# intel-aero/aero-optical-flow

Measured on AMD Instinct MI355X. Metric: frame-pairs/s (640x480, 8x8 SAD, +-4 search), higher is better.
Workload: dtype u8

## Files before the change

aero-optical-flow_amd/csrc/aof_batch.cpp:

```cpp
#include <cerrno>

#include "aof_batch_plan.hpp"
#include "aof_ctx.hpp"

using namespace aof;

namespace {

struct Timed {
    aof_ctx *ctx; int id; hipStream_t s; bool on; int slot;
    Timed(aof_ctx *c, int k, hipStream_t st)
        : ctx(c), id(k), s(st), on(c->prof.on && !c->capturing && ((c->prof.mask >> k) & 1u)),
          slot((int)(c->prof.count[k] % AOF_PROFILE_RING))
    {
        if (on) (void)hipEventRecord(ctx->prof.ev[id][slot][0], s);
    }
    ~Timed() { if (on) { (void)hipEventRecord(ctx->prof.ev[id][slot][1], s); ctx->prof.count[id]++; } }
};

VoteMem vote_mem(const aof_ctx *ctx) { return {ctx->votes.mem, kVoteStride, ctx->h_fault, ctx->votes.deadline_ticks}; }

int launch_lane8(aof_ctx *ctx, SearchArgs a, const FlowTail &tail, hipStream_t s, bool *reduced)
{
    hipStreamCaptureStatus status = hipStreamCaptureStatusNone;
    const Capture cap = hipStreamIsCapturing(s, &status) != hipSuccess ? CAPTURE_UNKNOWN
                        : status == hipStreamCaptureStatusNone         ? CAPTURE_NONE
                                                                       : CAPTURE_ACTIVE;
    const VoteMem vm = vote_mem(ctx);
    Lane8Launch l = choose_lane8(ctx->cfg, ctx->adapt, a, cap, vm, ctx->votes.pairs, ctx->votes.separate, ctx->votes.captured);
    a.prune = l.prune;
    const bool eager = cap == CAPTURE_NONE;
    if (l.fused && eager && ctx->votes.used && ctx->votes.stream != s && hipStreamWaitEvent(s, ctx->votes.done, 0) != hipSuccess)
// ... 167 lines not shown
```

aero-optical-flow_amd/csrc/aof_flow_small.hpp:

```cpp
#pragma once

#include "aof_device.hpp"
#include "aof_internal.hpp"
#include "aof_reduce.hpp"
#include "aof_refine.hpp"
#include "aof_sad.hpp"
#include "aof_small_plan.hpp"

namespace aof {

namespace {

__device__ __forceinline__ uint4 lds_bytes16(const uint8_t *frame, int off)
{
    const uint32_t *q = reinterpret_cast<const uint32_t *>(frame) + (off >> 2);
    const uint32_t sh = (uint32_t)off & 3u;
    const uint32_t q0 = q[0], q1 = q[1], q2 = q[2], q3 = q[3], q4 = q[4];
    return make_uint4(__builtin_amdgcn_alignbyte(q1, q0, sh), __builtin_amdgcn_alignbyte(q2, q1, sh),
                      __builtin_amdgcn_alignbyte(q3, q2, sh), __builtin_amdgcn_alignbyte(q4, q3, sh));
}
__device__ __forceinline__ void lds_bytes8(const uint8_t *frame, int off, uint32_t (&out)[2])
{
    const uint32_t *q = reinterpret_cast<const uint32_t *>(frame) + (off >> 2);
    const uint32_t sh = (uint32_t)off & 3u;
// ... 309 lines not shown
}

inline size_t small_lds_bytes(const SmallArgs &a) { return small_plan_make(a).lds; }

template <typename... Params, typename... Args>
inline int launch_small_class(void (*fn)(Params...), uint32_t grid, const SmallArgs &sm, void *stream, const Args &...args)
{
    const SmallPlan plan = small_plan_make(sm);
    if (plan.verdict != SMALL_OK) return (int)hipErrorInvalidValue;
    const size_t lds = plan.lds;
    if (plan.attr) {
        const hipError_t e = hipFuncSetAttribute(reinterpret_cast<const void *>(fn),
                                                 hipFuncAttributeMaxDynamicSharedMemorySize, (int)(kSmallLdsLimit - kSmallStaticLds));
        if (e != hipSuccess) return (int)e;
    }
    hipLaunchKernelGGL(fn, dim3(grid), dim3(kThreads), lds, static_cast<hipStream_t>(stream), args...);
    return (int)hipGetLastError();
}

}

}
```

aero-optical-flow_amd/csrc/k_coarse.hip:

```cpp
#include <cstdint>

#include "aof_coarse_plan.hpp"
#include "aof_device.hpp"
#include "aof_internal.hpp"
#include "aof_lab_hooks.hpp"
#include "aof_reduce.hpp"
#include "aof_sad.hpp"

namespace aof {

namespace {

constexpr int kThreads = 512;
constexpr int kUnroll = 4;
constexpr uint32_t kGated = 0xFFFFFFFEu;
constexpr uint32_t kOpen = 0xFFFFFFFFu;
constexpr int kMaxBins = 64;
constexpr int kNonTemporal = 2;
constexpr int kScratch = 8;
static_assert(kThreads == kCoarseThreads && kUnroll == kCoarseUnroll && kMaxBins == kCoarseMaxBins && kScratch == kCoarseScratch,
              "the kernel and its plan agree on the workgroup, the batches and the histograms");

__device__ __forceinline__ void lds_barrier()
{
// ... 257 lines not shown
        k.stagger_ticks = plan.stagger_ticks;
    }
    const size_t lds = plan.lds;
    const int64_t wgs = plan.wgs;
#ifdef AOF_LAB_COARSE_WS
    {
        int rc = 0;
        if (lab_launch_coarse_ws(k, wgs, lds, stream, &rc)) return rc;
    }
#endif
    {
        const hipError_t e = hipFuncSetAttribute(reinterpret_cast<const void *>(k_coarse),
                                                 hipFuncAttributeMaxDynamicSharedMemorySize, (int)kCoarseLdsLimit);
        if (e != hipSuccess) return (int)e;
    }
    hipLaunchKernelGGL(k_coarse, dim3((uint32_t)wgs), dim3(kThreads), lds, static_cast<hipStream_t>(stream), k);
    return (int)hipGetLastError();
}

}
```

aero-optical-flow_amd/csrc/k_cols8_flow_f.hip:

```cpp
#include "aof_cols8_kernels.hpp"
#include "aof_lane8_launch.hpp"

namespace aof {

int launch_k_flow_lane8_cols_f(const SearchArgs &a, const ColsPlan &plan, const PruneReport &rep, const ColsVotes &cv, uint32_t grid, int threads,
                               void *stream)
{
    hipLaunchKernelGGL((k_flow_lane8_cols<false>), dim3(grid), dim3(threads), 0, static_cast<hipStream_t>(stream), a, plan, rep, cv);
    return (int)hipGetLastError();
}

}
```

aero-optical-flow_amd/csrc/k_cols8_flow_t.hip:

```cpp
#include "aof_cols8_kernels.hpp"
#include "aof_lane8_launch.hpp"

namespace aof {

int launch_k_flow_lane8_cols_t(const SearchArgs &a, const ColsPlan &plan, const PruneReport &rep, const ColsVotes &cv, uint32_t grid, int threads,
                               void *stream)
{
    hipLaunchKernelGGL((k_flow_lane8_cols<true>), dim3(grid), dim3(threads), 0, static_cast<hipStream_t>(stream), a, plan, rep, cv);
    return (int)hipGetLastError();
}

}
```

aero-optical-flow_amd/csrc/k_cols8_search_f.hip:

```cpp
#include "aof_cols8_kernels.hpp"
#include "aof_lane8_launch.hpp"

namespace aof {

int launch_k_search_lane8_cols_f(const SearchArgs &a, const ColsPlan &plan, const PruneReport &rep, uint32_t wgs, int threads, void *stream)
{
    hipLaunchKernelGGL((k_search_lane8_cols<false>), dim3(wgs), dim3(threads), 0, static_cast<hipStream_t>(stream), a, plan, rep);
    return (int)hipGetLastError();
}

}
```

aero-optical-flow_amd/csrc/k_cols8_search_t.hip:

```cpp
#include "aof_cols8_kernels.hpp"
#include "aof_lane8_launch.hpp"

namespace aof {

int launch_k_search_lane8_cols_t(const SearchArgs &a, const ColsPlan &plan, const PruneReport &rep, uint32_t wgs, int threads, void *stream)
{
    hipLaunchKernelGGL((k_search_lane8_cols<true>), dim3(wgs), dim3(threads), 0, static_cast<hipStream_t>(stream), a, plan, rep);
    return (int)hipGetLastError();
}

}
```

aero-optical-flow_amd/csrc/k_lane8_flat_ff.hip:

```cpp
#include "aof_lane8_kernels.hpp"
#include "aof_lane8_launch.hpp"

namespace aof {

int launch_k_flow_lane8_flat_ff(const SearchArgs &a, uint32_t items, uint32_t search_wgs, uint32_t grid, int threads, const FlowTail &t,
                                const VoteMem &v, void *stream)
{
    hipLaunchKernelGGL((k_flow_lane8_flat<false, false>), dim3(grid), dim3(threads), 0, static_cast<hipStream_t>(stream), a, items, search_wgs, t, v);
    return (int)hipGetLastError();
}

}
```

aero-optical-flow_amd/csrc/k_lane8_flat_ft.hip:

```cpp
#include "aof_lane8_kernels.hpp"
#include "aof_lane8_launch.hpp"

namespace aof {

int launch_k_flow_lane8_flat_ft(const SearchArgs &a, uint32_t items, uint32_t search_wgs, uint32_t grid, int threads, const FlowTail &t,
                                const VoteMem &v, void *stream)
{
    hipLaunchKernelGGL((k_flow_lane8_flat<false, true>), dim3(grid), dim3(threads), 0, static_cast<hipStream_t>(stream), a, items, search_wgs, t, v);
    return (int)hipGetLastError();
}

}
```

aero-optical-flow_amd/csrc/k_lane8_flat_tf.hip:

```cpp
#include "aof_lane8_kernels.hpp"
#include "aof_lane8_launch.hpp"

namespace aof {

int launch_k_flow_lane8_flat_tf(const SearchArgs &a, uint32_t items, uint32_t search_wgs, uint32_t grid, int threads, const FlowTail &t,
                                const VoteMem &v, void *stream)
{
    hipLaunchKernelGGL((k_flow_lane8_flat<true, false>), dim3(grid), dim3(threads), 0, static_cast<hipStream_t>(stream), a, items, search_wgs, t, v);
    return (int)hipGetLastError();
}

}
```

aero-optical-flow_amd/csrc/k_lane8_flat_tt.hip:

```cpp
#include "aof_lane8_kernels.hpp"
#include "aof_lane8_launch.hpp"

namespace aof {

int launch_k_flow_lane8_flat_tt(const SearchArgs &a, uint32_t items, uint32_t search_wgs, uint32_t grid, int threads, const FlowTail &t,
                                const VoteMem &v, void *stream)
{
    hipLaunchKernelGGL((k_flow_lane8_flat<true, true>), dim3(grid), dim3(threads), 0, static_cast<hipStream_t>(stream), a, items, search_wgs, t, v);
    return (int)hipGetLastError();
}

}
```

aero-optical-flow_amd/csrc/k_lane8_group_f.hip:

```cpp
#include "aof_lane8_kernels.hpp"
#include "aof_lane8_launch.hpp"

namespace aof {

int launch_k_flow_lane8_f(const SearchArgs &a, const FlowTail &t, int ppw, uint32_t wgs, size_t lds, void *stream)
{
    hipLaunchKernelGGL((k_flow_lane8<false>), dim3(wgs), dim3(kThreads), lds, static_cast<hipStream_t>(stream), a, t, ppw);
    return (int)hipGetLastError();
}

}
```

aero-optical-flow_amd/csrc/k_lane8_group_t.hip:

```cpp
#include "aof_lane8_kernels.hpp"
#include "aof_lane8_launch.hpp"

namespace aof {

int launch_k_flow_lane8_t(const SearchArgs &a, const FlowTail &t, int ppw, uint32_t wgs, size_t lds, void *stream)
{
    hipLaunchKernelGGL((k_flow_lane8<true>), dim3(wgs), dim3(kThreads), lds, static_cast<hipStream_t>(stream), a, t, ppw);
    return (int)hipGetLastError();
}

}
```

aero-optical-flow_amd/csrc/k_lane8_pruned_f.hip:

```cpp
#include "aof_lane8_kernels.hpp"
#include "aof_lane8_launch.hpp"

namespace aof {

int launch_k_search_lane8_pruned_f(const SearchArgs &a, uint32_t items, uint32_t wgs, int spw, const PruneReport &rep, void *stream)
{
    hipLaunchKernelGGL((k_search_lane8_pruned<false>), dim3(wgs), dim3(kThreads), 0, static_cast<hipStream_t>(stream), a, items, wgs, spw, rep);
    return (int)hipGetLastError();
}

}
```

aero-optical-flow_amd/csrc/k_lane8_pruned_t.hip:

```cpp
#include "aof_lane8_kernels.hpp"
#include "aof_lane8_launch.hpp"

namespace aof {

int launch_k_search_lane8_pruned_t(const SearchArgs &a, uint32_t items, uint32_t wgs, int spw, const PruneReport &rep, void *stream)
{
    hipLaunchKernelGGL((k_search_lane8_pruned<true>), dim3(wgs), dim3(kThreads), 0, static_cast<hipStream_t>(stream), a, items, wgs, spw, rep);
    return (int)hipGetLastError();
}

}
```

aero-optical-flow_amd/csrc/k_lane8_search_ff.hip:

```cpp
#include "aof_lane8_kernels.hpp"
#include "aof_lane8_launch.hpp"

namespace aof {

int launch_k_search_lane8_ff(const SearchArgs &a, uint32_t items, uint32_t wgs, int threads, void *stream)
{
    hipLaunchKernelGGL((k_search_lane8<false, false>), dim3(wgs), dim3(threads), 0, static_cast<hipStream_t>(stream), a, items, wgs, 1);
    return (int)hipGetLastError();
}

}
```

aero-optical-flow_amd/csrc/k_lane8_search_ft.hip:

```cpp
#include "aof_lane8_kernels.hpp"
#include "aof_lane8_launch.hpp"

namespace aof {

int launch_k_search_lane8_ft(const SearchArgs &a, uint32_t items, uint32_t wgs, int threads, void *stream)
{
    hipLaunchKernelGGL((k_search_lane8<false, true>), dim3(wgs), dim3(threads), 0, static_cast<hipStream_t>(stream), a, items, wgs, 1);
    return (int)hipGetLastError();
}

}
```

aero-optical-flow_amd/csrc/k_lane8_search_tf.hip:

```cpp
#include "aof_lane8_kernels.hpp"
#include "aof_lane8_launch.hpp"

namespace aof {

int launch_k_search_lane8_tf(const SearchArgs &a, uint32_t items, uint32_t wgs, int threads, void *stream)
{
    hipLaunchKernelGGL((k_search_lane8<true, false>), dim3(wgs), dim3(threads), 0, static_cast<hipStream_t>(stream), a, items, wgs, 1);
    return (int)hipGetLastError();
}

}
```

aero-optical-flow_amd/csrc/k_lane8_search_tt.hip:

```cpp
#include "aof_lane8_kernels.hpp"
#include "aof_lane8_launch.hpp"

namespace aof {

int launch_k_search_lane8_tt(const SearchArgs &a, uint32_t items, uint32_t wgs, int threads, void *stream)
{
    hipLaunchKernelGGL((k_search_lane8<true, true>), dim3(wgs), dim3(threads), 0, static_cast<hipStream_t>(stream), a, items, wgs, 1);
    return (int)hipGetLastError();
}

}
```

aero-optical-flow_amd/csrc/k_pyramid.hip:

```cpp
#include "aof_coarse_plan.hpp"
#include "aof_device.hpp"
#include "aof_internal.hpp"

namespace aof {

namespace {

constexpr int kThreads = 256;
static_assert(kThreads == kPyramidThreads, "the kernels and their plan agree on the workgroup");

__device__ __forceinline__ void publish_sums(const PyramidArgs &a, int64_t unit, int frame, uint32_t sum0, uint32_t sum1)
{
    if (!a.sequence) {
        atomicAdd(&a.sums[unit * 4 + frame * 2 + 0], sum0);
        atomicAdd(&a.sums[unit * 4 + frame * 2 + 1], sum1);
        return;
    }
    if (unit < a.n_pairs - 1) {
        atomicAdd(&a.sums[unit * 4 + 0], sum0);
        atomicAdd(&a.sums[unit * 4 + 1], sum1);
    }
    if (unit > 0) {
        atomicAdd(&a.sums[(unit - 1) * 4 + 2], sum0);
        atomicAdd(&a.sums[(unit - 1) * 4 + 3], sum1);
// ... 82 lines not shown
}

__global__ __launch_bounds__(kThreads) void k_zero_words(uint32_t *words, int64_t count)
{
    const int64_t i = (int64_t)blockIdx.x * kThreads + threadIdx.x;
    if (i < count) words[i] = 0;
}

}

int launch_zero_words(uint32_t *words, int64_t count, void *stream)
{
    if (count <= 0) return 0;
    const int64_t wgs = (count + kThreads - 1) / kThreads;
    if (wgs > 0x7FFFFFFF) return (int)hipErrorInvalidValue;
    hipLaunchKernelGGL(k_zero_words, dim3((uint32_t)wgs), dim3(kThreads), 0, static_cast<hipStream_t>(stream), words, count);
    return (int)hipGetLastError();
}

int launch_pyramid(const PyramidArgs &a, void *stream)
{
    if (a.n_pairs == 0) return 0;
    hipStream_t s = static_cast<hipStream_t>(stream);
    const PyramidPlan plan = pyramid_plan_make(a.w, a.h, a.pair_stride, reinterpret_cast<uintptr_t>(a.prev), reinterpret_cast<uintptr_t>(a.cur),
                                               a.sequence, a.n_pairs, a.sums != nullptr);
    if (a.sums) {
        const int rc = launch_zero_words(a.sums, plan.zero_words, stream);
        if (rc) return rc;
    }
    if (plan.total > 0x7FFFFFFF) return (int)hipErrorInvalidValue;
    if (plan.vec)
        hipLaunchKernelGGL(k_pyramid_vec, dim3((uint32_t)plan.total), dim3(kThreads), 0, s, a, plan.rows_per_strip, plan.nstrips);
    else
        hipLaunchKernelGGL(k_pyramid_scalar, dim3((uint32_t)plan.total), dim3(kThreads), 0, s, a, plan.nstrips);
    return (int)hipGetLastError();
}

}
```

aero-optical-flow_amd/csrc/k_reduce.hip:

```cpp
#include "aof_device.hpp"
#include "aof_internal.hpp"
#include "aof_reduce.hpp"

namespace aof {

namespace {

constexpr int kThreads = 256;
constexpr int kMaxHist = 256;
constexpr int64_t kMidPairs = 1024;
constexpr int64_t kWidePairs = 512;

template <int GROUP, int kThreads = 256>
__global__ __launch_bounds__(kThreads) void k_reduce(ReduceArgs a)
{
    constexpr int kGroups = kThreads / GROUP;
    __shared__ uint32_t s_hist[kGroups][2][kMaxHist];
    __shared__ int s_sums[kGroups][3];
    const int grp = (int)threadIdx.x / GROUP, tid = (int)threadIdx.x % GROUP;
    const int64_t pair = (int64_t)blockIdx.x * kGroups + grp;
    if (GROUP < kThreads && pair >= a.n_pairs) return;
    auto sync = [] { if (GROUP == kThreads) __syncthreads(); else __builtin_amdgcn_wave_barrier(); };
    uint32_t (*hist)[kMaxHist] = s_hist[grp];
    int *sums = s_sums[grp];
    const int centre = 2 * a.tail.range + 1, n = 2 * centre + 1;
    for (int k = tid; k < n; k += GROUP) { hist[0][k] = 0; hist[1][k] = 0; }
    if (tid < 3) sums[tid] = 0;
    sync();

    if (a.parts) {
        const uint32_t *parts = a.parts + (size_t)pair * a.nstrips * (size_t)(2 * n);
        for (int k = tid; k < 2 * n; k += GROUP) {
            uint32_t v = 0;
            for (int st = 0; st < a.nstrips; st++) v += parts[(size_t)st * (2 * n) + k];
            const int axis = k >= n, bin = k - axis * n;
            hist[axis][bin] = v;
// ... 125 lines not shown
        wave_vote(hist[1], 2 * r.dy + hy + centre, ok);
    }
    __syncthreads();
    uint32_t *out = a.chunk_parts + ((size_t)pair * chunks + chunk) * (size_t)(2 * n);
    for (int k = tid; k < 2 * n; k += kThreads) out[k] = k < n ? hist[0][k] : hist[1][k - n];
}

}

int launch_reduce(const ReduceArgs &a, void *stream)
{
    if (a.n_pairs == 0) return 0;
    if (a.n_pairs > 0x7FFFFFFF) return (int)hipErrorInvalidValue;
    const int chunks = a.parts ? 0 : reduce_chunks(a.tail.nblocks);
    if (chunks > 0 && a.chunk_parts && a.n_pairs * chunks <= 0x7FFFFFFF) {
        hipLaunchKernelGGL(k_reduce_chunk, dim3((uint32_t)(a.n_pairs * chunks)), dim3(kThreads), 0,
                           static_cast<hipStream_t>(stream), a, chunks);
        ReduceArgs b = a;
        b.parts = a.chunk_parts;
        b.nstrips = chunks;
        hipLaunchKernelGGL(k_reduce<kThreads>, dim3((uint32_t)a.n_pairs), dim3(kThreads), 0,
                           static_cast<hipStream_t>(stream), b);
        return (int)hipGetLastError();
    }
    if (a.tail.nblocks <= 256 && !a.parts)
        hipLaunchKernelGGL(k_reduce<64>, dim3((uint32_t)((a.n_pairs + 3) / 4)), dim3(kThreads), 0,
                           static_cast<hipStream_t>(stream), a);
    else if (a.n_pairs <= kWidePairs && a.tail.nblocks >= 2048 && !a.parts)
        hipLaunchKernelGGL((k_reduce<1024, 1024>), dim3((uint32_t)a.n_pairs), dim3(1024), 0,
                           static_cast<hipStream_t>(stream), a);
    else if (a.n_pairs <= kMidPairs && a.tail.nblocks >= 2048 && !a.parts)
        hipLaunchKernelGGL((k_reduce<512, 512>), dim3((uint32_t)a.n_pairs), dim3(512), 0,
                           static_cast<hipStream_t>(stream), a);
    else
        hipLaunchKernelGGL(k_reduce<kThreads>, dim3((uint32_t)a.n_pairs), dim3(kThreads), 0,
                           static_cast<hipStream_t>(stream), a);
    return (int)hipGetLastError();
}

}
```

aero-optical-flow_amd/csrc/k_refine.hip:

```cpp
#include "aof_device.hpp"
#include "aof_internal.hpp"
#include "aof_refine.hpp"

namespace aof {

namespace {

constexpr int kRefineThreads = 256;

template <int NW>
__global__ __launch_bounds__(kRefineThreads) void k_refine(SearchArgs a, int64_t items)
{
    constexpr int B = 4 * NW;
    const int64_t item = (int64_t)blockIdx.x * kRefineThreads + threadIdx.x;
    if (item >= items) return;
    const int nb = a.grid.blocks();
    const int64_t pair = item / nb;
    const int blk = (int)(item - pair * nb);
    const aof_block rec = __builtin_bit_cast(
        aof_block, reinterpret_cast<const uint32_t *>(a.blocks)[pair * nb + blk]);
    uint8_t *out = a.subdirs + pair * nb + blk;
    if (rec.sad == AOF_SAD_SKIPPED || (uint32_t)rec.sad >= (uint32_t)a.value_threshold) {
        *out = 8;
        return;
// ... 41 lines not shown
    });
    const int subdir = st.direction(rec.sad);
    *out = (uint8_t)subdir;
}

}

int launch_refine(const SearchArgs &a, void *stream)
{
    if (a.n_pairs == 0 || !a.subdirs) return 0;
    const int64_t items = a.n_pairs * a.grid.blocks();
    const int64_t wgs = (items + kRefineThreads - 1) / kRefineThreads;
    if (wgs > 0x7FFFFFFF) return (int)hipErrorInvalidValue;
    const dim3 grid((uint32_t)wgs);
    if (a.tile == 8)
        hipLaunchKernelGGL(k_refine<2>, grid, dim3(kRefineThreads), 0, static_cast<hipStream_t>(stream), a, items);
    else if (a.tile == 16)
        hipLaunchKernelGGL(k_refine<4>, grid, dim3(kRefineThreads), 0, static_cast<hipStream_t>(stream), a, items);
    else
        return (int)hipErrorInvalidValue;
    return (int)hipGetLastError();
}

}
```

aero-optical-flow_amd/csrc/k_search_generic.hip:

```cpp
#include "aof_device.hpp"
#include "aof_internal.hpp"

namespace aof {

namespace {

constexpr int kMaxTile = 16, kMaxSearch = 8;
constexpr int kMaxWin = kMaxTile + 2 * kMaxSearch + 2;
constexpr int kMaxPitch = (kMaxWin + 3) / 4 * 4;

__global__ __launch_bounds__(64) void k_search_generic(SearchArgs a)
{
    __shared__ __attribute__((aligned(16))) uint8_t s_ref[kMaxTile * kMaxTile];
    __shared__ __attribute__((aligned(16))) uint8_t s_win[kMaxPitch * kMaxWin + 16];

    const int lane = threadIdx.x;
    const int blk = blockIdx.x;
    const int64_t pair = blockIdx.y + (int64_t)blockIdx.z * gridDim.y;
    if (pair >= a.n_pairs) return;
    const int B = a.tile, S = a.search, m = a.subpixel ? 1 : 0;
    const int bx = blk % a.grid.nx, by = blk / a.grid.nx;
    const int i = a.grid.x0 + bx * a.grid.step_x, j = a.grid.y0 + by * a.grid.step_y;
    int px = 0, py = 0;
    if (a.pred) { px = a.pred[pair].pred_x; py = a.pred[pair].pred_y; }
// ... 100 lines not shown
        }
    }
    if (lane == 0) {
        *out = rec;
        if (out_sd) *out_sd = (uint8_t)subdir;
    }
}

}

int launch_search_generic(const SearchArgs &a, void *stream)
{
    if (a.n_pairs == 0) return 0;
    const int64_t gy = a.n_pairs < 32768 ? a.n_pairs : 32768;
    const int64_t gz = (a.n_pairs + gy - 1) / gy;
    hipLaunchKernelGGL(k_search_generic, dim3((uint32_t)a.grid.blocks(), (uint32_t)gy, (uint32_t)gz),
                       dim3(64), 0, static_cast<hipStream_t>(stream), a);
    return (int)hipGetLastError();
}

}
```

aero-optical-flow_amd/csrc/k_search_tile16.hip:

```cpp
#include "aof_device.hpp"
#include "aof_internal.hpp"
#include "aof_refine.hpp"
#include "aof_sad.hpp"
#include "aof_tile16_plan.hpp"

namespace aof {

namespace {

constexpr int kBoundRows = 2;
constexpr uint32_t kFullOverBound = 6;
constexpr uint32_t kMaxSurvivorsPct = 35;
constexpr uint32_t kFullOverOneRow = 12;
constexpr uint32_t kMaxOneRowSurvivorsPct = 4;
constexpr uint32_t kMaxFourRowSurvivorsPct = 40, kMaxEightRowSurvivorsPct = 10;
constexpr uint32_t kMaxSeparationForDeeperLook = 450;
constexpr int kRefineParts = 4;

template <int NR, int STEP>
__device__ __forceinline__ void sum_item(const uint8_t *s_prev, const uint8_t *s_cur, int W, int dyi, int bx, int xs,
                                         int first, u64 (&acc)[4], uint32_t &acc16, int delta = 0)
{
    uint32_t ref[NR][4];
#pragma unroll
// ... 496 lines not shown
constexpr uint32_t kForcedVerdictPattern = 0x5A5A00u;
__global__ __launch_bounds__(kFillThreads) void k_tile16_fill_verdicts(uint32_t *hints, int64_t n_pairs, Tile16Verdicts f)
{
    const int64_t i = (int64_t)blockIdx.x * kFillThreads + threadIdx.x;
    if (i < n_pairs) hints[i] = (uint32_t)f.v[i % f.count] | kForcedVerdictPattern;
}

}

int launch_search_tile16(const SearchArgs &a, void *stream, const Tile16Verdicts &forced)
{
    if (a.n_pairs == 0) return 0;
    const Tile16Plan p = tile16_plan(a, forced.count);
    if (p.refused) return (int)hipErrorInvalidValue;
    if (p.front == TILE16_FRONT_FILL) {
        hipLaunchKernelGGL(k_tile16_fill_verdicts, dim3((uint32_t)p.front_wgs), dim3(kFillThreads), 0, static_cast<hipStream_t>(stream), a.hints,
                           a.n_pairs, forced);
    } else if (p.front == TILE16_FRONT_PROBE) {
        hipLaunchKernelGGL(k_tile16_probe, dim3((uint32_t)p.front_wgs), dim3(kProbeThreads), 0, static_cast<hipStream_t>(stream), a, a.hints,
                           p.stx, p.sty);
    }
    if (p.front != TILE16_FRONT_NONE) {
        const hipError_t e = hipGetLastError();
        if (e != hipSuccess) return (int)e;
    }
    SearchArgs k = a;
    k.div_nx = fastdiv_make((uint32_t)a.grid.nx);
    void (*fn)(SearchArgs, uint32_t) =
        p.refine ? (p.prune ? k_search_tile16<true, true> : k_search_tile16<false, true>)
                 : (p.prune ? k_search_tile16<true, false> : k_search_tile16<false, false>);
    if (p.attr) {
        hipError_t e = hipFuncSetAttribute(reinterpret_cast<const void *>(fn), hipFuncAttributeMaxDynamicSharedMemorySize, (int)p.lds);
        if (e != hipSuccess) return (int)e;
    }
    hipLaunchKernelGGL(fn, dim3((uint32_t)p.total), dim3(kTile16Threads), p.lds, static_cast<hipStream_t>(stream), k, (uint32_t)p.total);
    return (int)hipGetLastError();
}

}
```

Measured before the change: 7.266 million.

## Route launches through profiling-aware wrapper and add bin-based per-pair reduce path

Adds a launch_kernel wrapper that, when profiling is active, records start/stop events inside the kernel launch via hipExtLaunchKernelGGL instead of issuing separate hipEventRecord calls, and converts all launch sites to it. Separately adds a reduce_pair_bins path in k_reduce for the full-workgroup case, voting into per-lane x/y bins with a weighted fast path when all four records in a quad agree. This is meant to avoid the shared-memory histogram work when the search range is small. The change also disables profiling during stream capture.

After: 7.427 million (median of 6 runs). 2.2% higher.

```diff
diff --git a/aero-optical-flow_amd/csrc/aof_batch.cpp b/aero-optical-flow_amd/csrc/aof_batch.cpp
--- a/aero-optical-flow_amd/csrc/aof_batch.cpp
+++ b/aero-optical-flow_amd/csrc/aof_batch.cpp
@@ -2,6 +2,7 @@
 
 #include "aof_batch_plan.hpp"
 #include "aof_ctx.hpp"
+#include "aof_launch.hpp"
 
 using namespace aof;
 
@@ -9,13 +10,29 @@
 
 struct Timed {
     aof_ctx *ctx; int id; hipStream_t s; bool on; int slot;
+    LaunchScope scope;
     Timed(aof_ctx *c, int k, hipStream_t st)
         : ctx(c), id(k), s(st), on(c->prof.on && !c->capturing && ((c->prof.mask >> k) & 1u)),
           slot((int)(c->prof.count[k] % AOF_PROFILE_RING))
     {
-        if (on) (void)hipEventRecord(ctx->prof.ev[id][slot][0], s);
-    }
-    ~Timed() { if (on) { (void)hipEventRecord(ctx->prof.ev[id][slot][1], s); ctx->prof.count[id]++; } }
+        hipStreamCaptureStatus status = hipStreamCaptureStatusNone;
+        if (on && (hipStreamIsCapturing(s, &status) != hipSuccess || status != hipStreamCaptureStatusNone)) on = false;
+        if (!on) return;
+        scope = {ctx->prof.ev[id][slot][0], ctx->prof.ev[id][slot][1], 0};
+        t_launch_scope = &scope;
+    }
+    ~Timed()
+    {
+        if (!on) return;
+        t_launch_scope = nullptr;
+        if (scope.launches == 0) {
+            (void)hipEventRecord(scope.start, s);
+            (void)hipEventRecord(scope.stop, s);
+        }
+        ctx->prof.count[id]++;
+    }
+    Timed(const Timed &) = delete;
+    Timed &operator=(const Timed &) = delete;
 };
 
 VoteMem vote_mem(const aof_ctx *ctx) { return {ctx->votes.mem, kVoteStride, ctx->h_fault, ctx->votes.deadline_ticks}; }
diff --git a/aero-optical-flow_amd/csrc/aof_flow_small.hpp b/aero-optical-flow_amd/csrc/aof_flow_small.hpp
--- a/aero-optical-flow_amd/csrc/aof_flow_small.hpp
+++ b/aero-optical-flow_amd/csrc/aof_flow_small.hpp
@@ -5,6 +5,7 @@
 #include "aof_reduce.hpp"
 #include "aof_refine.hpp"
 #include "aof_sad.hpp"
+#include "aof_launch.hpp"
 #include "aof_small_plan.hpp"
 
 namespace aof {
@@ -347,7 +348,7 @@
                                                  hipFuncAttributeMaxDynamicSharedMemorySize, (int)(kSmallLdsLimit - kSmallStaticLds));
         if (e != hipSuccess) return (int)e;
     }
-    hipLaunchKernelGGL(fn, dim3(grid), dim3(kThreads), lds, static_cast<hipStream_t>(stream), args...);
+    launch_kernel(fn, dim3(grid), dim3(kThreads), lds, static_cast<hipStream_t>(stream), args...);
     return (int)hipGetLastError();
 }
 
diff --git a/aero-optical-flow_amd/csrc/aof_launch.hpp b/aero-optical-flow_amd/csrc/aof_launch.hpp
--- /dev/null
+++ b/aero-optical-flow_amd/csrc/aof_launch.hpp
@@ -0,0 +1,36 @@
+#pragma once
+
+#include <hip/hip_runtime.h>
+
+namespace aof {
+
+struct LaunchScope {
+    hipEvent_t start, stop;
+    int launches;
+};
+
+inline thread_local LaunchScope *t_launch_scope = nullptr;
+
+}
+
+#if defined(__HIP__)
+#include <hip/hip_ext.h>
+
+namespace aof {
+
+template <typename... Params, typename... Args>
+inline void launch_kernel(void (*kernel)(Params...), dim3 grid, dim3 block, size_t lds, hipStream_t stream, const Args &...args)
+{
+    static_assert(sizeof...(Params) == sizeof...(Args), "one argument per kernel parameter");
+    LaunchScope *sc = t_launch_scope;
+    if (!sc) {
+        hipLaunchKernelGGL(kernel, grid, block, (uint32_t)lds, stream, static_cast<Params>(args)...);
+        return;
+    }
+    hipExtLaunchKernelGGL(kernel, grid, block, (uint32_t)lds, stream, sc->launches == 0 ? sc->start : nullptr, sc->stop, 0u,
+                          static_cast<Params>(args)...);
+    sc->launches++;
+}
+
+}
+#endif
diff --git a/aero-optical-flow_amd/csrc/k_coarse.hip b/aero-optical-flow_amd/csrc/k_coarse.hip
--- a/aero-optical-flow_amd/csrc/k_coarse.hip
+++ b/aero-optical-flow_amd/csrc/k_coarse.hip
@@ -6,6 +6,7 @@
 #include "aof_lab_hooks.hpp"
 #include "aof_reduce.hpp"
 #include "aof_sad.hpp"
+#include "aof_launch.hpp"
 
 namespace aof {
 
@@ -295,7 +296,7 @@
                                                  hipFuncAttributeMaxDynamicSharedMemorySize, (int)kCoarseLdsLimit);
         if (e != hipSuccess) return (int)e;
     }
-    hipLaunchKernelGGL(k_coarse, dim3((uint32_t)wgs), dim3(kThreads), lds, static_cast<hipStream_t>(stream), k);
+    launch_kernel(k_coarse, dim3((uint32_t)wgs), dim3(kThreads), lds, static_cast<hipStream_t>(stream), k);
     return (int)hipGetLastError();
 }
 
diff --git a/aero-optical-flow_amd/csrc/k_cols8_flow_f.hip b/aero-optical-flow_amd/csrc/k_cols8_flow_f.hip
--- a/aero-optical-flow_amd/csrc/k_cols8_flow_f.hip
+++ b/aero-optical-flow_amd/csrc/k_cols8_flow_f.hip
@@ -1,12 +1,13 @@
 #include "aof_cols8_kernels.hpp"
 #include "aof_lane8_launch.hpp"
+#include "aof_launch.hpp"
 
 namespace aof {
 
 int launch_k_flow_lane8_cols_f(const SearchArgs &a, const ColsPlan &plan, const PruneReport &rep, const ColsVotes &cv, uint32_t grid, int threads,
                                void *stream)
 {
-    hipLaunchKernelGGL((k_flow_lane8_cols<false>), dim3(grid), dim3(threads), 0, static_cast<hipStream_t>(stream), a, plan, rep, cv);
+    launch_kernel((k_flow_lane8_cols<false>), dim3(grid), dim3(threads), 0, static_cast<hipStream_t>(stream), a, plan, rep, cv);
     return (int)hipGetLastError();
 }
 
diff --git a/aero-optical-flow_amd/csrc/k_cols8_flow_t.hip b/aero-optical-flow_amd/csrc/k_cols8_flow_t.hip
--- a/aero-optical-flow_amd/csrc/k_cols8_flow_t.hip
+++ b/aero-optical-flow_amd/csrc/k_cols8_flow_t.hip
@@ -1,12 +1,13 @@
 #include "aof_cols8_kernels.hpp"
 #include "aof_lane8_launch.hpp"
+#include "aof_launch.hpp"
 
 namespace aof {
 
 int launch_k_flow_lane8_cols_t(const SearchArgs &a, const ColsPlan &plan, const PruneReport &rep, const ColsVotes &cv, uint32_t grid, int threads,
                                void *stream)
 {
-    hipLaunchKernelGGL((k_flow_lane8_cols<true>), dim3(grid), dim3(threads), 0, static_cast<hipStream_t>(stream), a, plan, rep, cv);
+    launch_kernel((k_flow_lane8_cols<true>), dim3(grid), dim3(threads), 0, static_cast<hipStream_t>(stream), a, plan, rep, cv);
     return (int)hipGetLastError();
 }
 
diff --git a/aero-optical-flow_amd/csrc/k_cols8_search_f.hip b/aero-optical-flow_amd/csrc/k_cols8_search_f.hip
--- a/aero-optical-flow_amd/csrc/k_cols8_search_f.hip
+++ b/aero-optical-flow_amd/csrc/k_cols8_search_f.hip
@@ -1,11 +1,12 @@
 #include "aof_cols8_kernels.hpp"
 #include "aof_lane8_launch.hpp"
+#include "aof_launch.hpp"
 
 namespace aof {
 
 int launch_k_search_lane8_cols_f(const SearchArgs &a, const ColsPlan &plan, const PruneReport &rep, uint32_t wgs, int threads, void *stream)
 {
-    hipLaunchKernelGGL((k_search_lane8_cols<false>), dim3(wgs), dim3(threads), 0, static_cast<hipStream_t>(stream), a, plan, rep);
+    launch_kernel((k_search_lane8_cols<false>), dim3(wgs), dim3(threads), 0, static_cast<hipStream_t>(stream), a, plan, rep);
     return (int)hipGetLastError();
 }
 
diff --git a/aero-optical-flow_amd/csrc/k_cols8_search_t.hip b/aero-optical-flow_amd/csrc/k_cols8_search_t.hip
--- a/aero-optical-flow_amd/csrc/k_cols8_search_t.hip
+++ b/aero-optical-flow_amd/csrc/k_cols8_search_t.hip
@@ -1,11 +1,12 @@
 #include "aof_cols8_kernels.hpp"
 #include "aof_lane8_launch.hpp"
+#include "aof_launch.hpp"
 
 namespace aof {
 
 int launch_k_search_lane8_cols_t(const SearchArgs &a, const ColsPlan &plan, const PruneReport &rep, uint32_t wgs, int threads, void *stream)
 {
-    hipLaunchKernelGGL((k_search_lane8_cols<true>), dim3(wgs), dim3(threads), 0, static_cast<hipStream_t>(stream), a, plan, rep);
+    launch_kernel((k_search_lane8_cols<true>), dim3(wgs), dim3(threads), 0, static_cast<hipStream_t>(stream), a, plan, rep);
     return (int)hipGetLastError();
 }
 
diff --git a/aero-optical-flow_amd/csrc/k_lane8_flat_ff.hip b/aero-optical-flow_amd/csrc/k_lane8_flat_ff.hip
--- a/aero-optical-flow_amd/csrc/k_lane8_flat_ff.hip
+++ b/aero-optical-flow_amd/csrc/k_lane8_flat_ff.hip
@@ -1,12 +1,13 @@
 #include "aof_lane8_kernels.hpp"
 #include "aof_lane8_launch.hpp"
+#include "aof_launch.hpp"
 
 namespace aof {
 
 int launch_k_flow_lane8_flat_ff(const SearchArgs &a, uint32_t items, uint32_t search_wgs, uint32_t grid, int threads, const FlowTail &t,
                                 const VoteMem &v, void *stream)
 {
-    hipLaunchKernelGGL((k_flow_lane8_flat<false, false>), dim3(grid), dim3(threads), 0, static_cast<hipStream_t>(stream), a, items, search_wgs, t, v);
+    launch_kernel((k_flow_lane8_flat<false, false>), dim3(grid), dim3(threads), 0, static_cast<hipStream_t>(stream), a, items, search_wgs, t, v);
     return (int)hipGetLastError();
 }
 
diff --git a/aero-optical-flow_amd/csrc/k_lane8_flat_ft.hip b/aero-optical-flow_amd/csrc/k_lane8_flat_ft.hip
--- a/aero-optical-flow_amd/csrc/k_lane8_flat_ft.hip
+++ b/aero-optical-flow_amd/csrc/k_lane8_flat_ft.hip
@@ -1,12 +1,13 @@
 #include "aof_lane8_kernels.hpp"
 #include "aof_lane8_launch.hpp"
+#include "aof_launch.hpp"
 
 namespace aof {
 
 int launch_k_flow_lane8_flat_ft(const SearchArgs &a, uint32_t items, uint32_t search_wgs, uint32_t grid, int threads, const FlowTail &t,
                                 const VoteMem &v, void *stream)
 {
-    hipLaunchKernelGGL((k_flow_lane8_flat<false, true>), dim3(grid), dim3(threads), 0, static_cast<hipStream_t>(stream), a, items, search_wgs, t, v);
+    launch_kernel((k_flow_lane8_flat<false, true>), dim3(grid), dim3(threads), 0, static_cast<hipStream_t>(stream), a, items, search_wgs, t, v);
     return (int)hipGetLastError();
 }
 
diff --git a/aero-optical-flow_amd/csrc/k_lane8_flat_tf.hip b/aero-optical-flow_amd/csrc/k_lane8_flat_tf.hip
--- a/aero-optical-flow_amd/csrc/k_lane8_flat_tf.hip
+++ b/aero-optical-flow_amd/csrc/k_lane8_flat_tf.hip
@@ -1,12 +1,13 @@
 #include "aof_lane8_kernels.hpp"
 #include "aof_lane8_launch.hpp"
+#include "aof_launch.hpp"
 
 namespace aof {
 
 int launch_k_flow_lane8_flat_tf(const SearchArgs &a, uint32_t items, uint32_t search_wgs, uint32_t grid, int threads, const FlowTail &t,
                                 const VoteMem &v, void *stream)
 {
-    hipLaunchKernelGGL((k_flow_lane8_flat<true, false>), dim3(grid), dim3(threads), 0, static_cast<hipStream_t>(stream), a, items, search_wgs, t, v);
+    launch_kernel((k_flow_lane8_flat<true, false>), dim3(grid), dim3(threads), 0, static_cast<hipStream_t>(stream), a, items, search_wgs, t, v);
     return (int)hipGetLastError();
 }
 
diff --git a/aero-optical-flow_amd/csrc/k_lane8_flat_tt.hip b/aero-optical-flow_amd/csrc/k_lane8_flat_tt.hip
--- a/aero-optical-flow_amd/csrc/k_lane8_flat_tt.hip
+++ b/aero-optical-flow_amd/csrc/k_lane8_flat_tt.hip
@@ -1,12 +1,13 @@
 #include "aof_lane8_kernels.hpp"
 #include "aof_lane8_launch.hpp"
+#include "aof_launch.hpp"
 
 namespace aof {
 
 int launch_k_flow_lane8_flat_tt(const SearchArgs &a, uint32_t items, uint32_t search_wgs, uint32_t grid, int threads, const FlowTail &t,
                                 const VoteMem &v, void *stream)
 {
-    hipLaunchKernelGGL((k_flow_lane8_flat<true, true>), dim3(grid), dim3(threads), 0, static_cast<hipStream_t>(stream), a, items, search_wgs, t, v);
+    launch_kernel((k_flow_lane8_flat<true, true>), dim3(grid), dim3(threads), 0, static_cast<hipStream_t>(stream), a, items, search_wgs, t, v);
     return (int)hipGetLastError();
 }
 
diff --git a/aero-optical-flow_amd/csrc/k_lane8_group_f.hip b/aero-optical-flow_amd/csrc/k_lane8_group_f.hip
--- a/aero-optical-flow_amd/csrc/k_lane8_group_f.hip
+++ b/aero-optical-flow_amd/csrc/k_lane8_group_f.hip
@@ -1,11 +1,12 @@
 #include "aof_lane8_kernels.hpp"
 #include "aof_lane8_launch.hpp"
+#include "aof_launch.hpp"
 
 namespace aof {
 
 int launch_k_flow_lane8_f(const SearchArgs &a, const FlowTail &t, int ppw, uint32_t wgs, size_t lds, void *stream)
 {
-    hipLaunchKernelGGL((k_flow_lane8<false>), dim3(wgs), dim3(kThreads), lds, static_cast<hipStream_t>(stream), a, t, ppw);
+    launch_kernel((k_flow_lane8<false>), dim3(wgs), dim3(kThreads), lds, static_cast<hipStream_t>(stream), a, t, ppw);
     return (int)hipGetLastError();
 }
 
diff --git a/aero-optical-flow_amd/csrc/k_lane8_group_t.hip b/aero-optical-flow_amd/csrc/k_lane8_group_t.hip
--- a/aero-optical-flow_amd/csrc/k_lane8_group_t.hip
+++ b/aero-optical-flow_amd/csrc/k_lane8_group_t.hip
@@ -1,11 +1,12 @@
 #include "aof_lane8_kernels.hpp"
 #include "aof_lane8_launch.hpp"
+#include "aof_launch.hpp"
 
 namespace aof {
 
 int launch_k_flow_lane8_t(const SearchArgs &a, const FlowTail &t, int ppw, uint32_t wgs, size_t lds, void *stream)
 {
-    hipLaunchKernelGGL((k_flow_lane8<true>), dim3(wgs), dim3(kThreads), lds, static_cast<hipStream_t>(stream), a, t, ppw);
+    launch_kernel((k_flow_lane8<true>), dim3(wgs), dim3(kThreads), lds, static_cast<hipStream_t>(stream), a, t, ppw);
     return (int)hipGetLastError();
 }
 
diff --git a/aero-optical-flow_amd/csrc/k_lane8_pruned_f.hip b/aero-optical-flow_amd/csrc/k_lane8_pruned_f.hip
--- a/aero-optical-flow_amd/csrc/k_lane8_pruned_f.hip
+++ b/aero-optical-flow_amd/csrc/k_lane8_pruned_f.hip
@@ -1,11 +1,12 @@
 #include "aof_lane8_kernels.hpp"
 #include "aof_lane8_launch.hpp"
+#include "aof_launch.hpp"
 
 namespace aof {
 
 int launch_k_search_lane8_pruned_f(const SearchArgs &a, uint32_t items, uint32_t wgs, int spw, const PruneReport &rep, void *stream)
 {
-    hipLaunchKernelGGL((k_search_lane8_pruned<false>), dim3(wgs), dim3(kThreads), 0, static_cast<hipStream_t>(stream), a, items, wgs, spw, rep);
+    launch_kernel((k_search_lane8_pruned<false>), dim3(wgs), dim3(kThreads), 0, static_cast<hipStream_t>(stream), a, items, wgs, spw, rep);
     return (int)hipGetLastError();
 }
 
diff --git a/aero-optical-flow_amd/csrc/k_lane8_pruned_t.hip b/aero-optical-flow_amd/csrc/k_lane8_pruned_t.hip
--- a/aero-optical-flow_amd/csrc/k_lane8_pruned_t.hip
+++ b/aero-optical-flow_amd/csrc/k_lane8_pruned_t.hip
@@ -1,11 +1,12 @@
 #include "aof_lane8_kernels.hpp"
 #include "aof_lane8_launch.hpp"
+#include "aof_launch.hpp"
 
 namespace aof {
 
 int launch_k_search_lane8_pruned_t(const SearchArgs &a, uint32_t items, uint32_t wgs, int spw, const PruneReport &rep, void *stream)
 {
-    hipLaunchKernelGGL((k_search_lane8_pruned<true>), dim3(wgs), dim3(kThreads), 0, static_cast<hipStream_t>(stream), a, items, wgs, spw, rep);
+    launch_kernel((k_search_lane8_pruned<true>), dim3(wgs), dim3(kThreads), 0, static_cast<hipStream_t>(stream), a, items, wgs, spw, rep);
     return (int)hipGetLastError();
 }
 
diff --git a/aero-optical-flow_amd/csrc/k_lane8_search_ff.hip b/aero-optical-flow_amd/csrc/k_lane8_search_ff.hip
--- a/aero-optical-flow_amd/csrc/k_lane8_search_ff.hip
+++ b/aero-optical-flow_amd/csrc/k_lane8_search_ff.hip
@@ -1,11 +1,12 @@
 #include "aof_lane8_kernels.hpp"
 #include "aof_lane8_launch.hpp"
+#include "aof_launch.hpp"
 
 namespace aof {
 
 int launch_k_search_lane8_ff(const SearchArgs &a, uint32_t items, uint32_t wgs, int threads, void *stream)
 {
-    hipLaunchKernelGGL((k_search_lane8<false, false>), dim3(wgs), dim3(threads), 0, static_cast<hipStream_t>(stream), a, items, wgs, 1);
+    launch_kernel((k_search_lane8<false, false>), dim3(wgs), dim3(threads), 0, static_cast<hipStream_t>(stream), a, items, wgs, 1);
     return (int)hipGetLastError();
 }
 
diff --git a/aero-optical-flow_amd/csrc/k_lane8_search_ft.hip b/aero-optical-flow_amd/csrc/k_lane8_search_ft.hip
--- a/aero-optical-flow_amd/csrc/k_lane8_search_ft.hip
+++ b/aero-optical-flow_amd/csrc/k_lane8_search_ft.hip
@@ -1,11 +1,12 @@
 #include "aof_lane8_kernels.hpp"
 #include "aof_lane8_launch.hpp"
+#include "aof_launch.hpp"
 
 namespace aof {
 
 int launch_k_search_lane8_ft(const SearchArgs &a, uint32_t items, uint32_t wgs, int threads, void *stream)
 {
-    hipLaunchKernelGGL((k_search_lane8<false, true>), dim3(wgs), dim3(threads), 0, static_cast<hipStream_t>(stream), a, items, wgs, 1);
+    launch_kernel((k_search_lane8<false, true>), dim3(wgs), dim3(threads), 0, static_cast<hipStream_t>(stream), a, items, wgs, 1);
     return (int)hipGetLastError();
 }
 
diff --git a/aero-optical-flow_amd/csrc/k_lane8_search_tf.hip b/aero-optical-flow_amd/csrc/k_lane8_search_tf.hip
--- a/aero-optical-flow_amd/csrc/k_lane8_search_tf.hip
+++ b/aero-optical-flow_amd/csrc/k_lane8_search_tf.hip
@@ -1,11 +1,12 @@
 #include "aof_lane8_kernels.hpp"
 #include "aof_lane8_launch.hpp"
+#include "aof_launch.hpp"
 
 namespace aof {
 
 int launch_k_search_lane8_tf(const SearchArgs &a, uint32_t items, uint32_t wgs, int threads, void *stream)
 {
-    hipLaunchKernelGGL((k_search_lane8<true, false>), dim3(wgs), dim3(threads), 0, static_cast<hipStream_t>(stream), a, items, wgs, 1);
+    launch_kernel((k_search_lane8<true, false>), dim3(wgs), dim3(threads), 0, static_cast<hipStream_t>(stream), a, items, wgs, 1);
     return (int)hipGetLastError();
 }
 
diff --git a/aero-optical-flow_amd/csrc/k_lane8_search_tt.hip b/aero-optical-flow_amd/csrc/k_lane8_search_tt.hip
--- a/aero-optical-flow_amd/csrc/k_lane8_search_tt.hip
+++ b/aero-optical-flow_amd/csrc/k_lane8_search_tt.hip
@@ -1,11 +1,12 @@
 #include "aof_lane8_kernels.hpp"
 #include "aof_lane8_launch.hpp"
+#include "aof_launch.hpp"
 
 namespace aof {
 
 int launch_k_search_lane8_tt(const SearchArgs &a, uint32_t items, uint32_t wgs, int threads, void *stream)
 {
-    hipLaunchKernelGGL((k_search_lane8<true, true>), dim3(wgs), dim3(threads), 0, static_cast<hipStream_t>(stream), a, items, wgs, 1);
+    launch_kernel((k_search_lane8<true, true>), dim3(wgs), dim3(threads), 0, static_cast<hipStream_t>(stream), a, items, wgs, 1);
     return (int)hipGetLastError();
 }
 
diff --git a/aero-optical-flow_amd/csrc/k_pyramid.hip b/aero-optical-flow_amd/csrc/k_pyramid.hip
--- a/aero-optical-flow_amd/csrc/k_pyramid.hip
+++ b/aero-optical-flow_amd/csrc/k_pyramid.hip
@@ -1,6 +1,7 @@
 #include "aof_coarse_plan.hpp"
 #include "aof_device.hpp"
 #include "aof_internal.hpp"
+#include "aof_launch.hpp"
 
 namespace aof {
 
@@ -120,7 +121,7 @@
     if (count <= 0) return 0;
     const int64_t wgs = (count + kThreads - 1) / kThreads;
     if (wgs > 0x7FFFFFFF) return (int)hipErrorInvalidValue;
-    hipLaunchKernelGGL(k_zero_words, dim3((uint32_t)wgs), dim3(kThreads), 0, static_cast<hipStream_t>(stream), words, count);
+    launch_kernel(k_zero_words, dim3((uint32_t)wgs), dim3(kThreads), 0, static_cast<hipStream_t>(stream), words, count);
     return (int)hipGetLastError();
 }
 
@@ -136,9 +137,9 @@
     }
     if (plan.total > 0x7FFFFFFF) return (int)hipErrorInvalidValue;
     if (plan.vec)
-        hipLaunchKernelGGL(k_pyramid_vec, dim3((uint32_t)plan.total), dim3(kThreads), 0, s, a, plan.rows_per_strip, plan.nstrips);
+        launch_kernel(k_pyramid_vec, dim3((uint32_t)plan.total), dim3(kThreads), 0, s, a, plan.rows_per_strip, plan.nstrips);
     else
-        hipLaunchKernelGGL(k_pyramid_scalar, dim3((uint32_t)plan.total), dim3(kThreads), 0, s, a, plan.nstrips);
+        launch_kernel(k_pyramid_scalar, dim3((uint32_t)plan.total), dim3(kThreads), 0, s, a, plan.nstrips);
     return (int)hipGetLastError();
 }
 
diff --git a/aero-optical-flow_amd/csrc/k_reduce.hip b/aero-optical-flow_amd/csrc/k_reduce.hip
--- a/aero-optical-flow_amd/csrc/k_reduce.hip
+++ b/aero-optical-flow_amd/csrc/k_reduce.hip
@@ -1,6 +1,7 @@
 #include "aof_device.hpp"
 #include "aof_internal.hpp"
 #include "aof_reduce.hpp"
+#include "aof_launch.hpp"
 
 namespace aof {
 
@@ -10,6 +11,167 @@
 constexpr int kMaxHist = 256;
 constexpr int64_t kMidPairs = 1024;
 constexpr int64_t kWidePairs = 512;
+
+
+__device__ __forceinline__ void bins_vote(uint32_t &h, int bin, bool active)
+{
+    const int lane = (int)(threadIdx.x & 63);
+    unsigned long long todo = __ballot(active);
+    while (todo) {
+        const int b = __builtin_amdgcn_readlane(bin, __ffsll((long long)todo) - 1);
+        const unsigned long long same = __ballot(active && bin == b) & todo;
+        if (lane == b) h += (uint32_t)__popcll(same);
+        todo &= ~same;
+    }
+}
+
+__device__ __forceinline__ void bins_vote2(uint32_t &hx, uint32_t &hy, int bin_x, int bin_y, bool active)
+{
+    const int lane = (int)(threadIdx.x & 63);
+    const unsigned long long todo = __ballot(active);
+    if (todo == 0) return;
+    const int key = bin_x | (bin_y << 16);
+    const int k = __builtin_amdgcn_readlane(key, __ffsll((long long)todo) - 1);
+    if ((__ballot(active && key == k) & todo) == todo) {
+        const uint32_t c = (uint32_t)__popcll(todo);
+        if (lane == (k & 0xFFFF)) hx += c;
+        if (lane == (k >> 16)) hy += c;
+        return;
+    }
+    bins_vote(hx, bin_x, active);
+    bins_vote(hy, bin_y, active);
+}
+
+__device__ __forceinline__ void bins_vote_weighted(uint32_t &h, int bin, int weight, unsigned long long m1, unsigned long long m2,
+                                                   unsigned long long m3, unsigned long long m4)
+{
+    const int lane = (int)(threadIdx.x & 63);
+    unsigned long long todo = m1 | m2 | m3 | m4;
+    while (todo) {
+        const int b = __builtin_amdgcn_readlane(bin, __ffsll((long long)todo) - 1);
+        const unsigned long long same = __ballot(weight != 0 && bin == b) & todo;
+        const uint32_t total = (uint32_t)(__popcll(same & m1) + 2 * __popcll(same & m2) + 3 * __popcll(same & m3) + 4 * __popcll(same & m4));
+        if (lane == b) h += total;
+        todo &= ~same;
+    }
+}
+
+__device__ __forceinline__ void bins_vote2_weighted(uint32_t &hx, uint32_t &hy, int key, int weight)
+{
+    const int lane = (int)(threadIdx.x & 63);
+    const unsigned long long m1 = __ballot(weight == 1), m2 = __ballot(weight == 2), m3 = __ballot(weight == 3), m4 = __ballot(weight == 4);
+    const unsigned long long todo = m1 | m2 | m3 | m4;
+    if (todo == 0) return;
+    const int k = __builtin_amdgcn_readlane(key, __ffsll((long long)todo) - 1);
+    if ((__ballot(weight != 0 && key == k) & todo) == todo) {
+        const uint32_t total = (uint32_t)(__popcll(m1) + 2 * __popcll(m2) + 3 * __popcll(m3) + 4 * __popcll(m4));
+        if (lane == (k & 0xFFFF)) hx += total;
+        if (lane == (k >> 16)) hy += total;
+        return;
+    }
+    bins_vote_weighted(hx, key & 0xFFFF, weight, m1, m2, m3, m4);
+    bins_vote_weighted(hy, key >> 16, weight, m1, m2, m3, m4);
+}
+
+__device__ __forceinline__ void subdir_steps(int sd, int *hx, int *hy)
+{
+    *hx = (sd == 0 || sd == 1 || sd == 7) ? 1 : ((sd == 3 || sd == 4 || sd == 5) ? -1 : 0);
+    *hy = (sd == 1 || sd == 2 || sd == 3) ? 1 : ((sd == 5 || sd == 6 || sd == 7) ? -1 : 0);
+}
+
+template <int THREADS>
+__device__ __forceinline__ void reduce_pair_bins(const ReduceArgs &a, int64_t pair)
+{
+    constexpr int kWaves = THREADS / 64;
+    constexpr int kQuads = 2048 / THREADS;
+    __shared__ uint32_t s_part[kWaves][2][64];
+    const int tid = (int)threadIdx.x, lane = tid & 63, wave = tid >> 6;
+    const int centre = 2 * a.tail.range + 1;
+    const aof_block *blocks = a.blocks + pair * a.tail.nblocks;
+    const uint8_t *subdirs = a.subdirs ? a.subdirs + pair * a.tail.nblocks : nullptr;
+    typedef uint32_t u32_bytes __attribute__((aligned(1)));
+    const uint32_t *words = reinterpret_cast<const uint32_t *>(blocks);
+    const int quads = a.tail.nblocks / 4;
+    const int qrounds = (quads + THREADS - 1) / THREADS;
+
+    uint32_t rec[kQuads][4], sdir[kQuads];
+#pragma unroll
+    for (int k = 0; k < kQuads; k++) {
+        const int q = k * THREADS + tid;
+#pragma unroll
+        for (int j = 0; j < 4; j++) rec[k][j] = 0xFFFF0000u;
+        sdir[k] = 0x08080808u;
+        if (k < qrounds && q < quads) {
+            __builtin_memcpy(rec[k], words + 4 * q, 16);
+            if (subdirs) sdir[k] = *reinterpret_cast<const u32_bytes *>(subdirs + 4 * q);
+        }
+    }
+    const int b_tail = 4 * quads + tid;
+    const bool in_tail = b_tail < a.tail.nblocks;
+    uint32_t rec_tail = 0xFFFF0000u;
+    int sd_tail = 8;
+    if (in_tail) {
+        rec_tail = words[b_tail];
+        if (subdirs) sd_tail = subdirs[b_tail];
+    }
+
+    auto key_of = [&](uint32_t raw) {
+        int sx = 0, sy = 0;
+        if (subdirs) subdir_steps((int)(raw >> 16), &sx, &sy);
+        const int vx = 2 * (int)(int8_t)(raw & 0xFFu) + sx, vy = 2 * (int)(int8_t)((raw >> 8) & 0xFFu) + sy;
+        return (vx + centre) | ((vy + centre) << 16);
+    };
+    uint32_t hx = 0, hy = 0;
+#pragma unroll
+    for (int k = 0; k < kQuads; k++) {
+        if (k * THREADS + (tid & ~63) >= quads) break;
+        const bool have = k * THREADS + tid < quads;
+        uint32_t raw[4], first = 0;
+        int weight = 0;
+        bool ok[4], messy = false;
+#pragma unroll
+        for (int j = 0; j < 4; j++) {
+            const uint32_t w = rec[k][j], sad = w >> 16;
+            ok[j] = have && !(sad == AOF_SAD_SKIPPED || (int)sad >= a.value_threshold);
+            raw[j] = (w & 0xFFFFu) | (subdirs ? ((sdir[k] >> (8 * j)) & 0xFFu) << 16 : 0u);
+            if (ok[j]) {
+                if (weight == 0) first = raw[j];
+                else if (raw[j] != first) messy = true;
+                weight++;
+            }
+        }
+        if (__ballot(messy) == 0) {
+            bins_vote2_weighted(hx, hy, key_of(first), weight);
+        } else {
+#pragma unroll
+            for (int j = 0; j < 4; j++) {
+                const int key = key_of(raw[j]);
+                bins_vote2(hx, hy, key & 0xFFFF, key >> 16, ok[j]);
+            }
+        }
+    }
+    if (wave == 0) {
+        const uint32_t sad = rec_tail >> 16;
+        const bool ok = in_tail && !(sad == AOF_SAD_SKIPPED || (int)sad >= a.value_threshold);
+        int sx = 0, sy = 0;
+        if (subdirs) subdir_steps(sd_tail, &sx, &sy);
+        const int vx = 2 * (int)(int8_t)(rec_tail & 0xFFu) + sx, vy = 2 * (int)(int8_t)((rec_tail >> 8) & 0xFFu) + sy;
+        bins_vote2(hx, hy, vx + centre, vy + centre, ok);
+    }
+    s_part[wave][0][lane] = hx;
+    s_part[wave][1][lane] = hy;
+    __syncthreads();
+    if (wave != 0) return;
+#pragma unroll
+    for (int w = 1; w < kWaves; w++) { hx += s_part[w][0][lane]; hy += s_part[w][1][lane]; }
+    const int total = (int)wave_sum_u32(hx);
+    int sum2x = 0, sum2y = 0;
+    if (!a.tail.hist_filter) {
+        sum2x = (int)wave_sum_u32((uint32_t)((lane - centre) * (int)hx));
+        sum2y = (int)wave_sum_u32((uint32_t)((lane - centre) * (int)hy));
+    }
+    finalise_flow_wave_bins(a.tail, pair, hx, hy, sum2x, sum2y, total);
+}
 
 template <int GROUP, int kThreads = 256>
 __global__ __launch_bounds__(kThreads) void k_reduce(ReduceArgs a)
@@ -20,6 +182,12 @@
     const int grp = (int)threadIdx.x / GROUP, tid = (int)threadIdx.x % GROUP;
     const int64_t pair = (int64_t)blockIdx.x * kGroups + grp;
     if (GROUP < kThreads && pair >= a.n_pairs) return;
+    if constexpr (GROUP == kThreads) {
+        if (!a.parts && 2 * (2 * a.tail.range + 1) + 1 <= 64 && a.tail.nblocks <= 8192) {
+            reduce_pair_bins<kThreads>(a, pair);
+            return;
+        }
+    }
     auto sync = [] { if (GROUP == kThreads) __syncthreads(); else __builtin_amdgcn_wave_barrier(); };
     uint32_t (*hist)[kMaxHist] = s_hist[grp];
     int *sums = s_sums[grp];
@@ -175,26 +343,26 @@
     if (a.n_pairs > 0x7FFFFFFF) return (int)hipErrorInvalidValue;
     const int chunks = a.parts ? 0 : reduce_chunks(a.tail.nblocks);
     if (chunks > 0 && a.chunk_parts && a.n_pairs * chunks <= 0x7FFFFFFF) {
-        hipLaunchKernelGGL(k_reduce_chunk, dim3((uint32_t)(a.n_pairs * chunks)), dim3(kThreads), 0,
+        launch_kernel(k_reduce_chunk, dim3((uint32_t)(a.n_pairs * chunks)), dim3(kThreads), 0,
                            static_cast<hipStream_t>(stream), a, chunks);
         ReduceArgs b = a;
         b.parts = a.chunk_parts;
         b.nstrips = chunks;
-        hipLaunchKernelGGL(k_reduce<kThreads>, dim3((uint32_t)a.n_pairs), dim3(kThreads), 0,
+        launch_kernel(k_reduce<kThreads>, dim3((uint32_t)a.n_pairs), dim3(kThreads), 0,
                            static_cast<hipStream_t>(stream), b);
         return (int)hipGetLastError();
     }
     if (a.tail.nblocks <= 256 && !a.parts)
-        hipLaunchKernelGGL(k_reduce<64>, dim3((uint32_t)((a.n_pairs + 3) / 4)), dim3(kThreads), 0,
+        launch_kernel(k_reduce<64>, dim3((uint32_t)((a.n_pairs + 3) / 4)), dim3(kThreads), 0,
                            static_cast<hipStream_t>(stream), a);
     else if (a.n_pairs <= kWidePairs && a.tail.nblocks >= 2048 && !a.parts)
-        hipLaunchKernelGGL((k_reduce<1024, 1024>), dim3((uint32_t)a.n_pairs), dim3(1024), 0,
+        launch_kernel((k_reduce<1024, 1024>), dim3((uint32_t)a.n_pairs), dim3(1024), 0,
                            static_cast<hipStream_t>(stream), a);
     else if (a.n_pairs <= kMidPairs && a.tail.nblocks >= 2048 && !a.parts)
-        hipLaunchKernelGGL((k_reduce<512, 512>), dim3((uint32_t)a.n_pairs), dim3(512), 0,
+        launch_kernel((k_reduce<512, 512>), dim3((uint32_t)a.n_pairs), dim3(512), 0,
                            static_cast<hipStream_t>(stream), a);
     else
-        hipLaunchKernelGGL(k_reduce<kThreads>, dim3((uint32_t)a.n_pairs), dim3(kThreads), 0,
+        launch_kernel(k_reduce<kThreads>, dim3((uint32_t)a.n_pairs), dim3(kThreads), 0,
                            static_cast<hipStream_t>(stream), a);
     return (int)hipGetLastError();
 }
diff --git a/aero-optical-flow_amd/csrc/k_refine.hip b/aero-optical-flow_amd/csrc/k_refine.hip
--- a/aero-optical-flow_amd/csrc/k_refine.hip
+++ b/aero-optical-flow_amd/csrc/k_refine.hip
@@ -1,6 +1,7 @@
 #include "aof_device.hpp"
 #include "aof_internal.hpp"
 #include "aof_refine.hpp"
+#include "aof_launch.hpp"
 
 namespace aof {
 
@@ -79,9 +80,9 @@
     if (wgs > 0x7FFFFFFF) return (int)hipErrorInvalidValue;
     const dim3 grid((uint32_t)wgs);
     if (a.tile == 8)
-        hipLaunchKernelGGL(k_refine<2>, grid, dim3(kRefineThreads), 0, static_cast<hipStream_t>(stream), a, items);
+        launch_kernel(k_refine<2>, grid, dim3(kRefineThreads), 0, static_cast<hipStream_t>(stream), a, items);
     else if (a.tile == 16)
-        hipLaunchKernelGGL(k_refine<4>, grid, dim3(kRefineThreads), 0, static_cast<hipStream_t>(stream), a, items);
+        launch_kernel(k_refine<4>, grid, dim3(kRefineThreads), 0, static_cast<hipStream_t>(stream), a, items);
     else
         return (int)hipErrorInvalidValue;
     return (int)hipGetLastError();
diff --git a/aero-optical-flow_amd/csrc/k_search_generic.hip b/aero-optical-flow_amd/csrc/k_search_generic.hip
--- a/aero-optical-flow_amd/csrc/k_search_generic.hip
+++ b/aero-optical-flow_amd/csrc/k_search_generic.hip
@@ -1,5 +1,6 @@
 #include "aof_device.hpp"
 #include "aof_internal.hpp"
+#include "aof_launch.hpp"
 
 namespace aof {
 
@@ -138,7 +139,7 @@
     if (a.n_pairs == 0) return 0;
     const int64_t gy = a.n_pairs < 32768 ? a.n_pairs : 32768;
     const int64_t gz = (a.n_pairs + gy - 1) / gy;
-    hipLaunchKernelGGL(k_search_generic, dim3((uint32_t)a.grid.blocks(), (uint32_t)gy, (uint32_t)gz),
+    launch_kernel(k_search_generic, dim3((uint32_t)a.grid.blocks(), (uint32_t)gy, (uint32_t)gz),
                        dim3(64), 0, static_cast<hipStream_t>(stream), a);
     return (int)hipGetLastError();
 }
diff --git a/aero-optical-flow_amd/csrc/k_search_tile16.hip b/aero-optical-flow_amd/csrc/k_search_tile16.hip
--- a/aero-optical-flow_amd/csrc/k_search_tile16.hip
+++ b/aero-optical-flow_amd/csrc/k_search_tile16.hip
@@ -2,6 +2,7 @@
 #include "aof_internal.hpp"
 #include "aof_refine.hpp"
 #include "aof_sad.hpp"
+#include "aof_launch.hpp"
 #include "aof_tile16_plan.hpp"
 
 namespace aof {
@@ -534,10 +535,10 @@
     const Tile16Plan p = tile16_plan(a, forced.count);
     if (p.refused) return (int)hipErrorInvalidValue;
     if (p.front == TILE16_FRONT_FILL) {
-        hipLaunchKernelGGL(k_tile16_fill_verdicts, dim3((uint32_t)p.front_wgs), dim3(kFillThreads), 0, static_cast<hipStream_t>(stream), a.hints,
+        launch_kernel(k_tile16_fill_verdicts, dim3((uint32_t)p.front_wgs), dim3(kFillThreads), 0, static_cast<hipStream_t>(stream), a.hints,
                            a.n_pairs, forced);
     } else if (p.front == TILE16_FRONT_PROBE) {
-        hipLaunchKernelGGL(k_tile16_probe, dim3((uint32_t)p.front_wgs), dim3(kProbeThreads), 0, static_cast<hipStream_t>(stream), a, a.hints,
+        launch_kernel(k_tile16_probe, dim3((uint32_t)p.front_wgs), dim3(kProbeThreads), 0, static_cast<hipStream_t>(stream), a, a.hints,
                            p.stx, p.sty);
     }
     if (p.front != TILE16_FRONT_NONE) {
@@ -553,7 +554,7 @@
         hipError_t e = hipFuncSetAttribute(reinterpret_cast<const void *>(fn), hipFuncAttributeMaxDynamicSharedMemorySize, (int)p.lds);
         if (e != hipSuccess) return (int)e;
     }
-    hipLaunchKernelGGL(fn, dim3((uint32_t)p.total), dim3(kTile16Threads), p.lds, static_cast<hipStream_t>(stream), k, (uint32_t)p.total);
+    launch_kernel(fn, dim3((uint32_t)p.total), dim3(kTile16Threads), p.lds, static_cast<hipStream_t>(stream), k, (uint32_t)p.total);
     return (int)hipGetLastError();
 }
 
```
